# roboterax/humanoid-gym

Hardware: AMD Instinct MI355X
Metric: env-steps/s (XBot-L PPO, whole job) (higher is better)
Workload: dtype bf16

## Files before the change

humanoid-gym_amd/csrc/hgym_gae.hip:

```cpp
#include "hgym_common.hpp"

namespace hgym {

constexpr int GAE_ENVS = 16;
constexpr int GAE_PAD = 17;

template <bool BOOT>
__global__ __launch_bounds__(256) void gae_kernel(int T, int N, float* __restrict__ rewards,
                                                  const float* __restrict__ values, const uint8_t* __restrict__ dones,
                                                  const uint8_t* __restrict__ time_outs,
                                                  const float* __restrict__ last_values, float gamma, float lam,
                                                  float* __restrict__ returns, float* __restrict__ advantages,
                                                  double* __restrict__ stats) {
    __shared__ float s_r[64][GAE_PAD];
    __shared__ float s_v[65][GAE_PAD];
    __shared__ float s_d[64][GAE_PAD];
    __shared__ float s_carry[GAE_ENVS];
    __shared__ double s_sum[4][2];
    const int tid = threadIdx.x, lane = tid & 63, wave = tid >> 6;
    const int e0 = blockIdx.x * GAE_ENVS;
    const int nE = min(GAE_ENVS, N - e0);
    if (tid < GAE_ENVS) s_carry[tid] = 0.0f;
    double sum1 = 0.0, sum2 = 0.0;
    const int ntiles = (T + 63) / 64;
    for (int tile = ntiles - 1; tile >= 0; --tile) {
        const int t0 = tile * 64;
        const int nT = min(64, T - t0);
        __syncthreads();
        for (int i = tid; i < 65 * GAE_ENVS; i += 256) {
            const int t = i / GAE_ENVS, el = i % GAE_ENVS;
            if (el < nE) {
                const int tg = t0 + t;
                if (t < nT) {
                    const int64_t gi = (int64_t)tg * N + e0 + el;
                    const float v = values[gi];
                    float r = rewards[gi];
                    if (BOOT) {
                        const float to = (float)(time_outs[gi] != 0);
                        r = r + gamma * (v * to);
                        rewards[gi] = r;
                    }
                    s_r[t][el] = r;
                    s_d[t][el] = (float)dones[gi];
                    s_v[t][el] = v;
                } else if (t == nT) {
                    s_v[t][el] = (tg >= T) ? last_values[e0 + el] : values[(int64_t)tg * N + e0 + el];
                }
            }
        }
        __syncthreads();
        for (int q = 0; q < GAE_ENVS / 4; ++q) {
            const int el = wave * (GAE_ENVS / 4) + q;
            if (el >= nE) break;
            const bool valid = lane < nT;
            float a = 1.0f, b = 0.0f, v = 0.0f;
            if (valid) {
                v = s_v[lane][el];
                const float nt = 1.0f - s_d[lane][el];
                b = s_r[lane][el] + nt * gamma * s_v[lane + 1][el] - v;
                a = nt * gamma * lam;
            }
#pragma unroll
            for (int off = 1; off < 64; off <<= 1) {
                const float a2 = __shfl_down(a, off, 64);
                const float b2 = __shfl_down(b, off, 64);
                if (lane + off < 64) {
                    b = b + a * b2;
                    a = a * a2;
                }
            }
            const float carry = s_carry[el];
            const float adv_t = b + a * carry;
            const float ret = adv_t + v;
            const float adv = ret - v;
            const float head = __shfl(adv_t, 0, 64);
            if (valid) {
                s_r[lane][el] = ret;
                s_d[lane][el] = adv;
                sum1 += (double)adv;
                sum2 += (double)adv * (double)adv;
            }
            if (lane == 0) s_carry[el] = head;
        }
        __syncthreads();
        for (int i = tid; i < 64 * GAE_ENVS; i += 256) {
            const int t = i / GAE_ENVS, el = i % GAE_ENVS;
            if (t < nT && el < nE) {
                returns[(int64_t)(t0 + t) * N + e0 + el] = s_r[t][el];
                advantages[(int64_t)(t0 + t) * N + e0 + el] = s_d[t][el];
            }
        }
    }
#pragma unroll
    for (int off = 32; off > 0; off >>= 1) {
        sum1 += __shfl_down(sum1, off, 64);
        sum2 += __shfl_down(sum2, off, 64);
    }
    if (lane == 0) {
        s_sum[wave][0] = sum1;
        s_sum[wave][1] = sum2;
    }
    __syncthreads();
    __shared__ int s_last;
    double* __restrict__ part = stats + 4;
    unsigned int* cnt = reinterpret_cast<unsigned int*>(stats + 3);
    if (tid == 0) {
        part[2 * blockIdx.x] = s_sum[0][0] + s_sum[1][0] + s_sum[2][0] + s_sum[3][0];
        part[2 * blockIdx.x + 1] = s_sum[0][1] + s_sum[1][1] + s_sum[2][1] + s_sum[3][1];
        __builtin_amdgcn_fence(__ATOMIC_RELEASE, "agent");
        const unsigned int done = __hip_atomic_fetch_add(cnt, 1u, __ATOMIC_ACQ_REL, __HIP_MEMORY_SCOPE_AGENT);
        s_last = (done == gridDim.x - 1u) ? 1 : 0;
    }
    __syncthreads();
    if (s_last) {
        __builtin_amdgcn_fence(__ATOMIC_ACQUIRE, "agent");
        double a = 0.0, b = 0.0;
        for (int i = tid; i < (int)gridDim.x; i += 256) {
            a += part[2 * i];
            b += part[2 * i + 1];
        }
#pragma unroll
        for (int off = 32; off > 0; off >>= 1) {
            a += __shfl_down(a, off, 64);
            b += __shfl_down(b, off, 64);
        }
        __syncthreads();
        if (lane == 0) {
            s_sum[wave][0] = a;
            s_sum[wave][1] = b;
        }
        __syncthreads();
        if (tid == 0) {
            stats[0] = s_sum[0][0] + s_sum[1][0] + s_sum[2][0] + s_sum[3][0];
            stats[1] = s_sum[0][1] + s_sum[1][1] + s_sum[2][1] + s_sum[3][1];
            stats[2] = (double)T * (double)N;
            __hip_atomic_store(cnt, 0u, __ATOMIC_RELAXED, __HIP_MEMORY_SCOPE_AGENT);
        }
    }
}

__global__ __launch_bounds__(256) void adv_normalize_kernel(int64_t count, float* __restrict__ adv, const double* __restrict__ stats) {
    const double n = stats[2];
    const double mean_d = stats[0] / n;
    double var = (stats[1] - stats[0] * stats[0] / n) / (n - 1.0);
    if (var < 0.0) var = 0.0;
    const float mean = (float)mean_d;
    const float denom = (float)sqrt(var) + 1e-8f;
    for (int64_t i = (int64_t)blockIdx.x * blockDim.x + threadIdx.x; i < count; i += (int64_t)gridDim.x * blockDim.x)
        adv[i] = (adv[i] - mean) / denom;
}

__global__ __launch_bounds__(256) void store_step_kernel(int n, const float* __restrict__ rew, const float* __restrict__ values,
                                                         const uint8_t* __restrict__ time_outs, const uint8_t* __restrict__ dones,
                                                         float gamma, float* __restrict__ rewards_slot, uint8_t* __restrict__ dones_slot) {
    const int i = blockIdx.x * blockDim.x + threadIdx.x;
    if (i >= n) return;
    const float to = time_outs ? (float)(time_outs[i] != 0) : 0.0f;
    rewards_slot[i] = rew[i] + gamma * (values[i] * to);
    dones_slot[i] = dones[i] != 0;
}

HG_HD uint32_t perm_mix(uint32_t x) {
    x ^= x >> 16;
    x *= 0x7feb352du;
    x ^= x >> 15;
    x *= 0x846ca68bu;
    x ^= x >> 16;
    return x;
}
HG_HD uint64_t perm_key(uint64_t seed, uint64_t draw) { return (seed ^ (draw * 0x9e3779b97f4a7c15ull)) * 0xd1342543de82ef95ull + draw; }
HG_HD int64_t perm_index(int64_t i, int64_t n, int half_bits, uint32_t k0, uint32_t k1) {
    const uint32_t mask = (1u << half_bits) - 1u;
    uint64_t x = (uint64_t)i;
    do {
        uint32_t l = (uint32_t)(x >> half_bits) & mask, r = (uint32_t)x & mask;
#pragma unroll
        for (uint32_t round = 0; round < 6; ++round) {
            const uint32_t f = perm_mix(r ^ perm_mix(k0 + round * 0x9e3779b9u) ^ k1) & mask;
            const uint32_t t = l ^ f;
            l = r;
            r = t;
        }
        x = ((uint64_t)l << half_bits) | r;
    } while (x >= (uint64_t)n);
    return (int64_t)x;
}
__global__ __launch_bounds__(256) void randperm_kernel(int64_t n, int half_bits, uint32_t k0, uint32_t k1, int64_t* __restrict__ out) {
    for (int64_t i = (int64_t)blockIdx.x * blockDim.x + threadIdx.x; i < n; i += (int64_t)gridDim.x * blockDim.x)
        out[i] = perm_index(i, n, half_bits, k0, k1);
}

__global__ __launch_bounds__(256) void randperm_dev_kernel(int64_t n, int half_bits, uint64_t seed, const int64_t* __restrict__ draw_p,
                                                           int64_t* __restrict__ out) {
    const uint64_t draw = (uint64_t)draw_p[0];
    const uint64_t key = perm_key(seed, draw);
    const uint32_t k0 = (uint32_t)key, k1 = (uint32_t)(key >> 32);
    for (int64_t i = (int64_t)blockIdx.x * blockDim.x + threadIdx.x; i < n; i += (int64_t)gridDim.x * blockDim.x)
        out[i] = perm_index(i, n, half_bits, k0, k1);
}

}

using namespace hgym;

extern "C" {

int32_t hgym_randperm_dev(int64_t n, uint64_t seed, const int64_t* draw, int64_t* out, void* stream) {
    HG_REQUIRE(n > 0 && n <= ((int64_t)1 << 40), HGYM_E_SHAPE, "n=%lld", (long long)n);
    HG_REQUIRE(out && draw, HGYM_E_BADARG, "null pointer");
    int half_bits = 1;
    while (((int64_t)1 << (2 * half_bits)) < n) ++half_bits;
    const int blocks = (int)((n + 255) / 256 > 4096 ? 4096 : (n + 255) / 256);
    hipLaunchKernelGGL(randperm_dev_kernel, dim3(blocks), dim3(256), 0, (hipStream_t)stream, n, half_bits, seed, draw, out);
    HG_CHECK_LAUNCH("randperm_dev_kernel");
    return HGYM_OK;
}

int32_t hgym_randperm(int64_t n, uint64_t seed, uint64_t draw, int64_t* out, void* stream) {
    HG_REQUIRE(n > 0 && n <= ((int64_t)1 << 40), HGYM_E_SHAPE, "n=%lld", (long long)n);
    HG_REQUIRE(out, HGYM_E_BADARG, "null output");
    int half_bits = 1;
    while (((int64_t)1 << (2 * half_bits)) < n) ++half_bits;
    const uint64_t key = perm_key(seed, draw);
    const int blocks = (int)((n + 255) / 256 > 4096 ? 4096 : (n + 255) / 256);
    hipLaunchKernelGGL(randperm_kernel, dim3(blocks), dim3(256), 0, (hipStream_t)stream, n, half_bits, (uint32_t)key, (uint32_t)(key >> 32), out);
    HG_CHECK_LAUNCH("randperm_kernel");
    return HGYM_OK;
}

int32_t hgym_store_step(int32_t n, const float* rew, const float* values, const uint8_t* time_outs, const uint8_t* dones,
                        float gamma, float* rewards_slot, uint8_t* dones_slot, void* stream) {
    HG_REQUIRE(n > 0, HGYM_E_SHAPE, "n=%d", n);
    HG_REQUIRE(rew && values && dones && rewards_slot && dones_slot, HGYM_E_BADARG, "null pointer");
    hipLaunchKernelGGL(store_step_kernel, dim3(ceil_div(n, 256)), dim3(256), 0, (hipStream_t)stream, n, rew, values, time_outs, dones,
                       gamma, rewards_slot, dones_slot);
    HG_CHECK_LAUNCH("store_step_kernel");
    return HGYM_OK;
}

int32_t hgym_gae(int32_t T, int32_t n, const float* rewards, const float* values, const uint8_t* dones, const float* last_values,
                 float gamma, float lam, float* returns, float* advantages, double* stats, void* stream) {
    HG_REQUIRE(T > 0 && n > 0, HGYM_E_SHAPE, "T=%d n=%d", T, n);
    HG_REQUIRE(rewards && values && dones && last_values && returns && advantages && stats, HGYM_E_BADARG, "null pointer");
    prof_begin(HGYM_PROF_GAE, (hipStream_t)stream);
    hipLaunchKernelGGL(gae_kernel<false>, dim3(ceil_div(n, GAE_ENVS)), dim3(256), 0, (hipStream_t)stream, T, n, const_cast<float*>(rewards), values,
                       dones, nullptr, last_values, gamma, lam, returns, advantages, stats);
    prof_end(HGYM_PROF_GAE, (hipStream_t)stream, (double)T * n * 17.0);
    HG_CHECK_LAUNCH("gae_kernel");
    return HGYM_OK;
}

int32_t hgym_gae_bootstrap(int32_t T, int32_t n, float* rewards, const float* values, const uint8_t* dones, const uint8_t* time_outs,
                           const float* last_values, float gamma, float lam, float* returns, float* advantages, double* stats, void* stream) {
    HG_REQUIRE(T > 0 && n > 0, HGYM_E_SHAPE, "T=%d n=%d", T, n);
    HG_REQUIRE(rewards && values && dones && time_outs && last_values && returns && advantages && stats, HGYM_E_BADARG, "null pointer");
    prof_begin(HGYM_PROF_GAE, (hipStream_t)stream);
    hipLaunchKernelGGL(gae_kernel<true>, dim3(ceil_div(n, GAE_ENVS)), dim3(256), 0, (hipStream_t)stream, T, n, rewards, values, dones, time_outs,
                       last_values, gamma, lam, returns, advantages, stats);
    prof_end(HGYM_PROF_GAE, (hipStream_t)stream, (double)T * n * 22.0);
    HG_CHECK_LAUNCH("gae_kernel<bootstrap>");
    return HGYM_OK;
}

int32_t hgym_adv_normalize(int64_t count, float* advantages, const double* stats, void* stream) {
    HG_REQUIRE(count > 1, HGYM_E_SHAPE, "count=%lld", (long long)count);
    HG_REQUIRE(advantages && stats, HGYM_E_BADARG, "null pointer");
    const int blocks = (int)((count + 255) / 256 > 2048 ? 2048 : (count + 255) / 256);
    hipLaunchKernelGGL(adv_normalize_kernel, dim3(blocks), dim3(256), 0, (hipStream_t)stream, count, advantages, stats);
    HG_CHECK_LAUNCH("adv_normalize_kernel");
    return HGYM_OK;
}

}
```

humanoid-gym_amd/csrc/hgym_net.hip:

```cpp
#include <stdlib.h>

#include "hgym_gemm.hpp"
#include "hgym_fused.hpp"

namespace hgym {

int32_t launch_mlp_fb(const FwdArgs& fb, const FbLoss& fl, bool shadow, bool unclipped, int tiles, int nets, size_t lds, hipStream_t s);

struct LayerLayout {
    int K, N;
    int Kp, Ncp, N16, K16;
    int64_t w_off, b_off;
    int64_t Wp, WTp;
    int64_t X, XT, dY, dYT;
    int KBf, NBf, NBBf;
    int64_t Wf, WTf;
};

struct NetLayout {
    int L;
    bool fused;
    LayerLayout layer[HGYM_MAX_LAYERS];
    int64_t out_f32;
    int64_t X0b, Hb[3], dZb[4];
// ... 335 lines not shown
        } else {
#pragma unroll
            for (int j = 0; j < 16; ++j) {
                if (j >= A) continue;
                rowm[j] = a.mu[(int64_t)i * A + j];
                rowa[j] = a.b.actions[r * A + j];
                rowmo[j] = a.b.mu[r * A + j];
                rowso[j] = a.b.sigma[r * A + j];
            }
        }
#pragma unroll
        for (int j = 0; j < 16; ++j) {
            diff[j] = 0.0f;
            sg[j] = 1.0f;
            if (j >= A) continue;
            const float m = rowm[j];
            const float s = m * 0.0f + a.std_[j];
            const float act = rowa[j];
            const float mo = rowmo[j], so = rowso[j];
            const float d = act - m;
            diff[j] = d;
            sg[j] = s;
            lp += -(d * d) / (2.0f * s * s) - logf(s) - 0.9189385332046727f;
            ent += 0.5f + 0.9189385332046727f + logf(s);
            kl += logf(s / so + 1.e-5f) + (so * so + (mo - m) * (mo - m)) / (2.0f * (s * s)) - 0.5f;
        }
        const float ratio = expf(lp - lpold);
        const float s1 = -adv * ratio;
        const float s2 = -adv * clampf(ratio, 1.0f - a.clip, 1.0f + a.clip);
        const float surr = fmaxf(s1, s2);
        const float in_range = (ratio >= 1.0f - a.clip && ratio <= 1.0f + a.clip) ? 1.0f : 0.0f;
        const float w1 = s1 > s2 ? 1.0f : (s1 == s2 ? 0.5f : 0.0f);
        const float d_lp = (-adv) * (w1 + (1.0f - w1) * in_range) * invB * ratio;
        float vl, d_v;
        if constexpr (VU) {
            vl = (v - ret) * (v - ret);
            d_v = a.value_coef * invB * (2.0f * (v - ret));
        } else {
            const float vc = vold + clampf(v - vold, -a.clip, a.clip);
            const float l1 = (v - ret) * (v - ret), l2 = (vc - ret) * (vc - ret);
            vl = fmaxf(l1, l2);
            const float v_in = ((v - vold) >= -a.clip && (v - vold) <= a.clip) ? 1.0f : 0.0f;
            const float u1 = l1 > l2 ? 1.0f : (l1 == l2 ? 0.5f : 0.0f);
            d_v = a.value_coef * invB * (u1 * 2.0f * (v - ret) + (1.0f - u1) * 2.0f * (vc - ret) * v_in);
        }
#pragma unroll
        for (int j = 0; j < 16; ++j) {
            if (j >= A) continue;
            const float s = sg[j], d = diff[j];
            const float g_mu = d_lp * d / (s * s);
            const float g_sg = d_lp * (d * d / (s * s * s) - 1.0f / s) - (a.entropy_coef * invB) / s;
            if (j < 12) {
                acc[4 + j] = g_sg;
                acc[16 + j] = g_mu;
            }
            dmu[(int64_t)i * a.ld_dmu + j] = from_f32<T>(g_mu);
            dmuT[(int64_t)j * a.ld_t + i] = from_f32<T>(g_mu);
        }
        dval[(int64_t)i * a.ld_dval] = from_f32<T>(d_v);
        dvalT[i] = from_f32<T>(d_v);
        acc[0] = surr;
        acc[1] = vl;
        acc[2] = ent;
        acc[3] = kl;
        acc[28] = d_v;
    } else if (i < a.Bp) {
        for (int j = 0; j < A; ++j) dmuT[(int64_t)j * a.ld_t + i] = from_f32<T>(0.0f);
        dvalT[i] = from_f32<T>(0.0f);
    }
#pragma unroll
    for (int k = 0; k < LOSS_PARTIALS; ++k) {
        float s = acc[k];
#pragma unroll
        for (int off = 32; off > 0; off >>= 1) s += __shfl_down(s, off, 64);
        if ((threadIdx.x & 63) == 0) red[threadIdx.x >> 6][k] = s;
    }
    __syncthreads();
    if (threadIdx.x < LOSS_PARTIALS) a.partials[(int64_t)blockIdx.x * LOSS_PARTIALS + threadIdx.x] =
        red[0][threadIdx.x] + red[1][threadIdx.x] + red[2][threadIdx.x] + red[3][threadIdx.x];
}

__global__ __launch_bounds__(512) void ppo_scalars_kernel(const ScalArgs a) { ppo_scalars_block(a, threadIdx.x, blockDim.x); }

struct Segment {
    int64_t off;
    int rows, cols;
    int splits;
    void* Wp;
    int64_t ldw;
    void* WTp;
    int64_t ldwt;
    void* Wf;
    void* WTf;
    int KB, NBB;
};
struct SegTable {
    int n;
    Segment s[2 * HGYM_MAX_LAYERS * 2 + 1];
};

__global__ __launch_bounds__(256) void reduce_slabs_kernel(const SegTable tab, int64_t P, const float* __restrict__ slabs,
                                                           float* __restrict__ grads, double* __restrict__ opt) {
    __shared__ double red[4];
    const Segment& sg = tab.s[blockIdx.y];
    const int64_t n = (int64_t)sg.rows * sg.cols;
    const int64_t stride = (int64_t)gridDim.x * blockDim.x;
    double sq = 0.0;
    if (sg.splits == 0) {
        for (int64_t i = (int64_t)blockIdx.x * blockDim.x + threadIdx.x; i < n; i += stride) {
            const float g = grads[sg.off + i];
            sq += (double)g * (double)g;
        }
    } else {
        const bool vec = (P & 3) == 0 && (((uintptr_t)grads | (uintptr_t)slabs) & 15) == 0;
        const int64_t head = vec ? ((4 - (sg.off & 3)) & 3) < n ? ((4 - (sg.off & 3)) & 3) : n : n;
        const int64_t n4 = (n - head) >> 2, tail0 = head + 4 * n4;
        const int64_t base = sg.off + head;
        for (int64_t i = (int64_t)blockIdx.x * blockDim.x + threadIdx.x; i < n4; i += stride) {
            float4 acc = make_float4(0.f, 0.f, 0.f, 0.f);
            if (sg.splits == 8) {
                float4 v[8];
#pragma unroll
                for (int z = 0; z < 8; ++z) v[z] = *reinterpret_cast<const float4*>(slabs + (int64_t)z * P + base + 4 * i);
#pragma unroll
                for (int z = 0; z < 8; ++z) { acc.x += v[z].x; acc.y += v[z].y; acc.z += v[z].z; acc.w += v[z].w; }
            } else {
                for (int z = 0; z < sg.splits; ++z) {
                    const float4 v = *reinterpret_cast<const float4*>(slabs + (int64_t)z * P + base + 4 * i);
                    acc.x += v.x; acc.y += v.y; acc.z += v.z; acc.w += v.w;
                }
            }
            *reinterpret_cast<float4*>(grads + base + 4 * i) = acc;
            sq += (double)acc.x * (double)acc.x + (double)acc.y * (double)acc.y + (double)acc.z * (double)acc.z + (double)acc.w * (double)acc.w;
        }
        for (int64_t i = (int64_t)blockIdx.x * blockDim.x + threadIdx.x; i < head + (n - tail0); i += stride) {
            const int64_t e = i < head ? i : tail0 + (i - head);
            float s = 0.0f;
            for (int z = 0; z < sg.splits; ++z) s += slabs[(int64_t)z * P + sg.off + e];
            grads[sg.off + e] = s;
            sq += (double)s * (double)s;
        }
    }
#pragma unroll
    for (int off = 32; off > 0; off >>= 1) sq += __shfl_down(sq, off, 64);
    if ((threadIdx.x & 63) == 0) red[threadIdx.x >> 6] = sq;
    __syncthreads();
    if (threadIdx.x == 0) {
        double t = red[0] + red[1] + red[2] + red[3];
        t = __builtin_rint(t * 0x1p46) * 0x1p-46;
        if (t != 0.0) atomicAdd(&opt[9], t);
    }
}


__device__ __forceinline__ void apply_prologue(const HgymPPOConfig& p, const float* __restrict__ kl_slot, float inv_w, double* __restrict__ opt,
                                               int have_sq, double sq) {
    if (p.world_size > 1) opt[8] = (double)(kl_slot[0] * inv_w);
    if (opt[13] == opt[1] && opt[1] > 0.0) {
        if (have_sq >= 0) opt[9] = have_sq ? sq : 0.0;
        return;
    }
    if (p.adaptive_lr) opt[0] = adapt_lr(opt[0], (float)opt[8], p.desired_kl, p.lr_min, p.lr_max);
    const double t = opt[1] + 1.0;
    opt[1] = t;
    const bool cached = opt[13] == t;
    const double bc1 = 1.0 - (cached ? opt[14] : pow((double)p.beta1, t)), bc2 = 1.0 - (cached ? opt[15] : pow((double)p.beta2, t));
    opt[11] = (double)(float)(opt[0] / bc1);
    opt[12] = (double)(float)sqrt(bc2);
    opt[13] = t;
    if (have_sq >= 0) opt[9] = have_sq ? sq : 0.0;
}
__global__ void apply_prologue_kernel(const HgymPPOConfig p, const float* __restrict__ kl_slot, float inv_w, double* __restrict__ opt) {
    if (threadIdx.x != 0 || blockIdx.x != 0) return;
    apply_prologue(p, kl_slot, inv_w, opt, (p.world_size > 1 || !p.grad_norm_ready) ? 0 : -1, 0.0);
}

__global__ __launch_bounds__(256) void sqnorm_prologue_kernel(int64_t P, const float* __restrict__ g, float inv_w, const HgymPPOConfig p,
                                                              const float* __restrict__ kl_slot, double* __restrict__ opt,
                                                              double* __restrict__ part) {
    __shared__ double red[4];
    __shared__ unsigned int s_last;
    double s = 0.0;
    for (int64_t i = (int64_t)blockIdx.x * blockDim.x + threadIdx.x; i < P; i += (int64_t)gridDim.x * blockDim.x) {
        const float gi = g[i] * inv_w;
        s += (double)gi * (double)gi;
    }
#pragma unroll
    for (int off = 32; off > 0; off >>= 1) s += __shfl_down(s, off, 64);
    if ((threadIdx.x & 63) == 0) red[threadIdx.x >> 6] = s;
    __syncthreads();
    unsigned int* counter = reinterpret_cast<unsigned int*>(part + SQN_BLOCKS);
    if (threadIdx.x == 0) {
        part[blockIdx.x] = red[0] + red[1] + red[2] + red[3];
        __threadfence();
        s_last = atomicAdd(counter, 1u) == gridDim.x - 1u ? 1u : 0u;
    }
    __syncthreads();
    if (!s_last) return;
    __threadfence();
    double v = threadIdx.x < gridDim.x ? reinterpret_cast<const volatile double*>(part)[threadIdx.x] : 0.0;
#pragma unroll
    for (int off = 32; off > 0; off >>= 1) v += __shfl_down(v, off, 64);
    __syncthreads();
    if ((threadIdx.x & 63) == 0) red[threadIdx.x >> 6] = v;
    __syncthreads();
    if (threadIdx.x == 0) {
        *counter = 0u;
        apply_prologue(p, kl_slot, inv_w, opt, 1, red[0] + red[1] + red[2] + red[3]);
    }
}

template <typename T>
__device__ __forceinline__ void write_shadows(const Segment& sg, int r, int c, float w) {
    if (sg.Wp) {
        ((T*)sg.Wp)[(int64_t)r * sg.ldw + c] = from_f32<T>(w);
        if (sg.WTp) ((T*)sg.WTp)[(int64_t)c * sg.ldwt + r] = from_f32<T>(w);
    }
    if (sg.Wf) {
        ((T*)sg.Wf)[((((int64_t)(r >> 4) * sg.KB + (c >> 5)) * 64) + ((c & 31) >> 3) * 16 + (r & 15)) * 8 + (c & 7)] = from_f32<T>(w);
        ((T*)sg.WTf)[((((int64_t)(c >> 4) * sg.NBB + (r >> 5)) * 64) + ((r & 31) >> 3) * 16 + (c & 15)) * 8 + (r & 7)] = from_f32<T>(w);
    }
}

template <typename T>
__global__ __launch_bounds__(256) void adam_kernel(const SegTable tab, const HgymPPOConfig p, float* __restrict__ params,
                                                   float* __restrict__ grads, float* __restrict__ m_, float* __restrict__ v_,
                                                   float inv_w, double* __restrict__ opt) {
    const Segment& sg = tab.s[blockIdx.y];
    const int64_t n = (int64_t)sg.rows * sg.cols;
    const float total = (float)sqrt(opt[9]);
    float coef = p.max_grad_norm / (total + 1e-6f);
    coef = fminf(coef, 1.0f);
    if (blockIdx.x == 0 && blockIdx.y == 0 && threadIdx.x == 0) {
        opt[6] = (double)total;
        opt[13] = -1.0;
    }
    const float step_size = (float)opt[11], sqrt_bc2 = (float)opt[12];
    auto adam1 = [&](int64_t q) -> float {
        const float g = (grads[q] * inv_w) * coef;
        grads[q] = g;
        const float m = m_[q] * p.beta1 + (1.0f - p.beta1) * g;
        const float v = v_[q] * p.beta2 + (1.0f - p.beta2) * (g * g);
        m_[q] = m;
        v_[q] = v;
        const float denom = sqrtf(v) / sqrt_bc2 + p.adam_eps;
        const float w = params[q] + (-step_size * m) / denom;
        params[q] = w;
        return w;
    };
    for (int64_t i = (int64_t)blockIdx.x * blockDim.x + threadIdx.x; i < n; i += (int64_t)gridDim.x * blockDim.x) {
        const float w = adam1(sg.off + i);
        if (sg.Wp || sg.Wf) {
            const int r = (int)(i / sg.cols), c = (int)(i - (int64_t)r * sg.cols);
            write_shadows<T>(sg, r, c, w);
        }
    }
}

template <typename T>
__global__ __launch_bounds__(256) void sync_shadow_kernel(const SegTable tab, const float* __restrict__ params) {
    const Segment& sg = tab.s[blockIdx.y];
    if (!sg.Wp && !sg.Wf) return;
    const int64_t n = (int64_t)sg.rows * sg.cols;
    for (int64_t i = (int64_t)blockIdx.x * blockDim.x + threadIdx.x; i < n; i += (int64_t)gridDim.x * blockDim.x) {
        const int r = (int)(i / sg.cols), c = (int)(i - (int64_t)r * sg.cols);
        write_shadows<T>(sg, r, c, params[sg.off + i]);
    }
}

template <typename T, int BM, int BN, int WMs, int WNs>
static void launch_cfg(const GemmArgs& g, int splits, hipStream_t s) {
    constexpr int F = ((BM / 16) + (BN / 16)) * KSTAGE;
    constexpr size_t lds = (size_t)2 * F * 1024;
    (void)ensure_dynamic_lds(reinterpret_cast<const void*>(&gemm_nt_kernel<T, BM, BN, WMs, WNs>), lds, "gemm_nt_kernel");
    dim3 grid(ceil_div(g.N, BN), ceil_div(g.M, BM), splits);
    hipLaunchKernelGGL((gemm_nt_kernel<T, BM, BN, WMs, WNs>), grid, dim3(WMs * WNs * 64), lds, s, g);
}

template <typename T>
int32_t launch_gemm(const GemmArgs& g0, int splits, hipStream_t s) {
    GemmArgs g = g0;
    constexpr int SE = stage_elems<T>();
    HG_REQUIRE(g.K % SE == 0 && g.K > 0, HGYM_E_SHAPE, "gemm K=%d not a multiple of %d", g.K, SE);
    HG_REQUIRE(g.lda * (int64_t)sizeof(T) % 16 == 0 && g.ldb * (int64_t)sizeof(T) % 16 == 0, HGYM_E_SHAPE, "gemm operand rows must be 16-byte aligned");
    if (splits < 1) splits = 1;
    int stages = g.K / SE;
    if (splits > stages) splits = stages;
    const int per = ceil_div(stages, splits);
    splits = ceil_div(stages, per);
    g.k_chunk = per * SE;
    prof_begin(HGYM_PROF_GEMM, s);
    const int64_t t128 = (int64_t)ceil_div(g.M, 128) * ceil_div(g.N, 128) * splits;
    if (g.N <= 16) launch_cfg<T, 128, 16, 4, 1>(g, splits, s);
    else if (g.M <= 16) launch_cfg<T, 16, 128, 1, 4>(g, splits, s);
    else if (t128 >= 192) launch_cfg<T, 128, 128, 2, 2>(g, splits, s);
    else launch_cfg<T, 64, 64, 2, 2>(g, splits, s);
    prof_end(HGYM_PROF_GEMM, s, 2.0 * (double)g.M * (double)g.N * (double)g.K);
    HG_CHECK_LAUNCH("gemm_nt_kernel");
    return splits;
}

struct NetIO {
    const float* x;
    int64_t ldx;
    float* out;
    int64_t ldo;
};

static int64_t shadow_ld(const WsLayout& w, int which) { return (int64_t)w.net[which].layer[0].KBf * 32; }

static int32_t check_shadow(const WsLayout& w, const HgymObsShadow* sh) {
    if (!sh) return HGYM_OK;
    HG_REQUIRE((!sh->obs || (sh->ld_obs >= shadow_ld(w, 0) && sh->ld_obs % 8 == 0 && ((uintptr_t)sh->obs & 15) == 0)) &&
                   (!sh->priv || (sh->ld_priv >= shadow_ld(w, 1) && sh->ld_priv % 8 == 0 && ((uintptr_t)sh->priv & 15) == 0)),
               HGYM_E_SHAPE, "observation shadow: leading dimensions %lld / %lld (need >= %lld / %lld, multiples of 8, 16-byte aligned rows)",
               (long long)sh->ld_obs, (long long)sh->ld_priv, (long long)shadow_ld(w, 0), (long long)shadow_ld(w, 1));
    return HGYM_OK;
}

static size_t fwd_lds(const FwdArgs& a, int nets, int BM) {
    size_t lds = 0;
    for (int i = 0; i < nets; ++i) lds = std::max(lds, (size_t)fwd_lds_bytes(a.net[a.net0 + i], BM));
    return lds;
}

struct NetBase {
    const HgymNetConfig& cfg;
    const HgymNet& net;
    const WsLayout& w;
    hipStream_t s;
    char* ws;

    template <typename U> U* at(int64_t off) const { return reinterpret_cast<U*>(ws + off); }

    int split_count(const LayerLayout& y, int Mp) const {
        const int tiles = ceil_div(y.N, y.N <= 16 ? 16 : 128) * ceil_div(y.K, 128);
        int sp = ceil_div(512, tiles);
        if (sp > w.splits) sp = w.splits;
        const int stages = Mp / w.SE;
        if (sp > stages) sp = stages;
        if (sp < 1) sp = 1;
        const int per = ceil_div(stages, sp);
        return ceil_div(stages, per);
    }

    int rowsum_splits(int Mp, int* per_out = nullptr) const {
        const int chunks = ceil_div(Mp, 1024 * 16 / w.es);
        const int per = ceil_div(chunks, std::min(chunks, w.splits));
        if (per_out) *per_out = per;
        return ceil_div(chunks, per);
    }

    SegTable segments(int Mp) const {
        SegTable t;
        memset(&t, 0, sizeof(t));
        Segment& sd = t.s[t.n++];
        sd.off = 0;
        sd.rows = cfg.num_actions;
        sd.cols = 1;
        for (int which = 0; which < w.nnets; ++which) {
            const NetLayout& n = w.net[which];
            for (int l = 0; l < n.L; ++l) {
                const LayerLayout& y = n.layer[l];
                Segment& a = t.s[t.n++];
                a.off = y.w_off;
                a.rows = y.N;
                a.cols = y.K;
                if (n.fused) {
                    a.splits = Mp ? w.dw_splits : 0;
                    a.Wf = ws + y.Wf;
                    a.WTf = ws + y.WTf;
                    a.KB = y.KBf;
                    a.NBB = y.NBBf;
                } else {
                    a.splits = Mp ? split_count(y, Mp) : 0;
                    a.Wp = ws + y.Wp;
                    a.ldw = y.Kp;
                    a.WTp = ws + y.WTp;
                    a.ldwt = y.Ncp;
                }
                Segment& b = t.s[t.n++];
                b.off = y.b_off;
                b.rows = y.N;
                b.cols = 1;
                if (n.fused && Mp && (l < n.L - 1 || which == 2)) b.splits = w.dw_splits;
                if (!n.fused && Mp) b.splits = rowsum_splits(Mp);
            }
        }
        return t;
    }

    template <typename T>
    int32_t apply(const HgymPPOConfig& ppo, bool prologue_done) {
        prof_begin(HGYM_PROF_APPLY, s);
        const float inv_w = ppo.world_size > 1 ? (float)(1.0 / (double)ppo.world_size) : 1.0f;
        if (ppo.world_size > 1 || !ppo.grad_norm_ready)
            hipLaunchKernelGGL(sqnorm_prologue_kernel, dim3(SQN_BLOCKS), dim3(256), 0, s, w.P, net.grads, inv_w, ppo, net.grads + w.P, net.opt_state,
                               at<double>(w.sqn));
        else if (!prologue_done)
            hipLaunchKernelGGL(apply_prologue_kernel, dim3(1), dim3(64), 0, s, ppo, net.grads + w.P, inv_w, net.opt_state);
        const SegTable tab = segments(0);
        hipLaunchKernelGGL((adam_kernel<T>), dim3(256, tab.n), dim3(256), 0, s, tab, ppo, net.params, net.grads, net.adam_m, net.adam_v,
                           inv_w, net.opt_state);
        prof_end(HGYM_PROF_APPLY, s, (double)w.P * 36.0);
        HG_CHECK_LAUNCH("adam_kernel");
        return HGYM_OK;
    }

    template <typename T>
    int32_t sync_shadow() {
        const SegTable tab = segments(0);
        hipLaunchKernelGGL((sync_shadow_kernel<T>), dim3(64, tab.n), dim3(256), 0, s, tab, net.params);
        HG_CHECK_LAUNCH("sync_shadow_kernel");
        return HGYM_OK;
    }
};

template <typename T>
struct GemmPath : NetBase {
    int32_t forward(int which, int M, const float* x, int64_t ldx, const int64_t* idx, float* y_out, int64_t ld_out, bool train) {
        const NetLayout& n = w.net[which];
        HG_REQUIRE(M > 0 && M <= w.maxM, HGYM_E_SHAPE, "batch %d exceeds max_batch %lld", M, (long long)w.maxM);
        const LayerLayout& l0 = n.layer[0];
        const int64_t total = (int64_t)M * l0.K;
        hipLaunchKernelGGL((pack_rows_kernel<T>), dim3((int)std::min<int64_t>(ceil_div(total, 256), 4096)), dim3(256), 0, s, M, l0.K, x,
                           ldx, idx, at<T>(l0.X), (int64_t)l0.Kp);
        HG_CHECK_LAUNCH("pack_rows_kernel");
        const int Mp = (int)round_up(M, w.SE);
        for (int l = 0; l < n.L; ++l) {
            const LayerLayout& y = n.layer[l];
            const bool last = l == n.L - 1;
            if (train) {
                hipLaunchKernelGGL((transpose_kernel<T>), dim3(ceil_div(Mp, 64), ceil_div(y.K, 64)), dim3(256), 0, s, M, Mp, y.K,
                                   at<T>(y.X), (int64_t)y.Kp, at<T>(y.XT), w.Mp);
                HG_CHECK_LAUNCH("transpose_kernel");
            }
            GemmArgs g;
            memset(&g, 0, sizeof(g));
            g.A = at<T>(y.X);
            g.lda = y.Kp;
            g.rowsA = M;
            g.B = at<T>(y.Wp);
            g.ldb = y.Kp;
            g.rowsB = y.N16;
            g.M = M;
            g.N = y.N;
            g.K = y.Kp;
            g.bias = net.params + y.b_off;
            if (last) {
                g.Cf = y_out;
                g.ldcf = ld_out;
            } else {
                g.act = ACT_APPLY;
                g.fn = w.act;
                g.Ct = at<T>(n.layer[l + 1].X);
                g.ldct = n.layer[l + 1].Kp;
            }
            const int32_t rc = launch_gemm<T>(g, 1, s);
            if (rc < 0) return rc;
        }
        return HGYM_OK;
    }

    int32_t backward(int which, int M) {
        const NetLayout& n = w.net[which];
        const int Mp = (int)round_up(M, w.SE);
        for (int l = n.L - 1; l >= 0; --l) {
            const LayerLayout& y = n.layer[l];
            {
                GemmArgs g;
                memset(&g, 0, sizeof(g));
                g.A = at<T>(y.dYT);
                g.lda = w.Mp;
                g.rowsA = y.N16;
                g.B = at<T>(y.XT);
                g.ldb = w.Mp;
                g.rowsB = y.K16;
                g.M = y.N;
                g.N = y.K;
                g.K = Mp;
                g.Cf = at<float>(w.slabs) + y.w_off;
                g.ldcf = y.K;
                g.slab_stride = w.Ps;
                const int want = split_count(y, Mp);
                const int32_t got = launch_gemm<T>(g, want, s);
                if (got < 0) return got;
                HG_REQUIRE(got == want, HGYM_E_LAUNCH, "split-K mismatch %d vs %d", got, want);
                int per = 0;
                const int rs = rowsum_splits(Mp, &per);
                hipLaunchKernelGGL((rowsum_kernel<T>), dim3(rs, y.N), dim3(256), 0, s, Mp, per, at<T>(y.dYT), w.Mp,
                                   at<float>(w.slabs) + y.b_off, w.Ps);
                HG_CHECK_LAUNCH("rowsum_kernel");
            }
            if (l > 0) {
                const LayerLayout& p = n.layer[l - 1];
                GemmArgs g;
                memset(&g, 0, sizeof(g));
                g.A = at<T>(y.dY);
                g.lda = y.Ncp;
                g.rowsA = M;
                g.B = at<T>(y.WTp);
                g.ldb = y.Ncp;
                g.rowsB = y.K16;
                g.M = M;
                g.N = y.K;
                g.K = y.Ncp;
                g.aux = at<T>(y.X);
                g.ldaux = y.Kp;
                g.fn = w.act;
                g.Ct = at<T>(p.dY);
                g.ldct = p.Ncp;
                const int32_t rc = launch_gemm<T>(g, 1, s);
                if (rc < 0) return rc;
                hipLaunchKernelGGL((transpose_kernel<T>), dim3(ceil_div(Mp, 64), ceil_div(p.N, 64)), dim3(256), 0, s, M, Mp, p.N,
                                   at<T>(p.dY), (int64_t)p.Ncp, at<T>(p.dYT), w.Mp);
                HG_CHECK_LAUNCH("transpose_kernel");
            }
        }
        return HGYM_OK;
    }

    int32_t aux_grad(const HgymPPOConfig& ppo, const HgymBatch& b) {
        const NetLayout& n = w.net[2];
        const LayerLayout& last = n.layer[n.L - 1];
        const int B = b.B, No = last.N;
        float* y = at<float>(n.out_f32);
        int32_t rc = forward(2, B, b.obs, cfg.num_obs, b.idx, y, No, true);
        if (rc) return rc;
        const int Bp = (int)round_up(B, w.SE);
        hipLaunchKernelGGL((aux_mse_kernel<T>), dim3(ceil_div(Bp, 256)), dim3(256), 0, s, B, Bp, No, y, b.priv, (int64_t)cfg.num_priv,
                           cfg.aux_target_offset, b.idx, ppo.aux_coef, at<T>(last.dY), (int64_t)last.Ncp, at<T>(last.dYT), w.Mp,
                           net.opt_state);
        HG_CHECK_LAUNCH("aux_mse_kernel");
        return backward(2, B);
    }

    int32_t grad(const HgymPPOConfig& ppo, const HgymBatch& b, int part) {
        if (part == 1) return HGYM_OK;
        const int B = b.B, A = cfg.num_actions;
        float* mu = at<float>(w.net[0].out_f32);
        float* val = at<float>(w.net[1].out_f32);
        int32_t rc = forward(0, B, b.obs, cfg.num_obs, b.idx, mu, A, true);
        if (rc) return rc;
        rc = forward(1, B, b.priv, cfg.num_priv, b.idx, val, 1, true);
        if (rc) return rc;
        const int Bp = (int)round_up(B, w.SE);
        const int nblocks = ceil_div(Bp, 256);
        HG_REQUIRE(nblocks <= MAX_LOSS_BLOCKS, HGYM_E_UNSUPPORTED, "minibatch %d too large for the loss partial buffer", B);
        const LayerLayout& la = w.net[0].layer[w.net[0].L - 1];
        const LayerLayout& lc = w.net[1].layer[w.net[1].L - 1];
        LossArgs a;
        memset(&a, 0, sizeof(a));
        a.b = b;
        a.A = A;
        a.mu = mu;
        a.val = val;
// ... 534 lines not shown
```

Baseline: 43.16 million.

## Vectorize GAE kernel and flatten Adam grid with tiled fragment-shadow writes

Adds a GAE kernel that handles twice as many envs per 512-thread block and loads and stores rewards, values, dones and time-outs as float4/uint32 vectors. It writes per-virtual-block partial sums so the existing stats layout is kept. The Adam launch becomes a flat 1D grid sized per segment instead of a fixed 256-by-segments grid. For bf16 fragment-layout shadows it stages updated weights through LDS tiles and writes packed 16-byte fragments for both the weight and its transpose, replacing scattered element writes. Both paths fall back to the old kernels through env vars or when alignment checks fail, at the cost of extra code complexity and LDS use.

```diff
diff --git a/humanoid-gym_amd/csrc/hgym_gae.hip b/humanoid-gym_amd/csrc/hgym_gae.hip
--- a/humanoid-gym_amd/csrc/hgym_gae.hip
+++ b/humanoid-gym_amd/csrc/hgym_gae.hip
@@ -139,6 +139,161 @@
     }
 }
 
+constexpr int GAEV_ENVS = 2 * GAE_ENVS;
+constexpr int GAEV_PAD = GAEV_ENVS + 1;
+template <bool BOOT>
+__global__ __launch_bounds__(512) void gae_vec_kernel(int T, int N, float* __restrict__ rewards, const float* __restrict__ values,
+                                                      const uint8_t* __restrict__ dones, const uint8_t* __restrict__ time_outs,
+                                                      const float* __restrict__ last_values, float gamma, float lam,
+                                                      float* __restrict__ returns, float* __restrict__ advantages, double* __restrict__ stats) {
+    __shared__ float s_r[64][GAEV_PAD];
+    __shared__ float s_v[65][GAEV_PAD];
+    __shared__ float s_d[64][GAEV_PAD];
+    __shared__ float s_carry[GAEV_ENVS];
+    __shared__ double s_sum[8][2];
+    const int tid = threadIdx.x, lane = tid & 63, wave = tid >> 6;
+    const int e0 = blockIdx.x * GAEV_ENVS;
+    const int nE = min(GAEV_ENVS, N - e0);
+    const int nvirt = (N + GAE_ENVS - 1) / GAE_ENVS;
+    const int st = tid >> 3, sg = (tid & 7) * 4;
+    if (tid < GAEV_ENVS) s_carry[tid] = 0.0f;
+    double sum1 = 0.0, sum2 = 0.0;
+    const int ntiles = (T + 63) / 64;
+    for (int tile = ntiles - 1; tile >= 0; --tile) {
+        const int t0 = tile * 64;
+        const int nT = min(64, T - t0);
+        const bool mine = st < nT && sg < nE;
+        const int64_t gi = (int64_t)(t0 + st) * N + e0 + sg;
+        float4 r4 = make_float4(0.f, 0.f, 0.f, 0.f), v4 = r4, x4 = r4;
+        uint32_t d4 = 0, to4 = 0;
+        if (mine) {
+            v4 = *reinterpret_cast<const float4*>(values + gi);
+            r4 = *reinterpret_cast<const float4*>(rewards + gi);
+            d4 = *reinterpret_cast<const uint32_t*>(dones + gi);
+            if (BOOT) to4 = *reinterpret_cast<const uint32_t*>(time_outs + gi);
+        }
+        const bool next = tid < GAEV_ENVS / 4 && tid * 4 < nE;
+        if (next)
+            x4 = (t0 + nT >= T) ? *reinterpret_cast<const float4*>(last_values + e0 + tid * 4)
+                                : *reinterpret_cast<const float4*>(values + (int64_t)(t0 + nT) * N + e0 + tid * 4);
+        __syncthreads();
+        if (mine) {
+            const float rr[4] = {r4.x, r4.y, r4.z, r4.w}, vv[4] = {v4.x, v4.y, v4.z, v4.w};
+            float ro[4];
+#pragma unroll
+            for (int j = 0; j < 4; ++j) {
+                float r = rr[j];
+                if (BOOT) {
+                    const float to = (float)(((to4 >> (8 * j)) & 0xffu) != 0);
+                    r = r + gamma * (vv[j] * to);
+                }
+                ro[j] = r;
+                s_r[st][sg + j] = r;
+                s_d[st][sg + j] = (float)((d4 >> (8 * j)) & 0xffu);
+                s_v[st][sg + j] = vv[j];
+            }
+            if (BOOT) *reinterpret_cast<float4*>(rewards + gi) = make_float4(ro[0], ro[1], ro[2], ro[3]);
+        }
+        if (next) {
+            s_v[nT][tid * 4 + 0] = x4.x;
+            s_v[nT][tid * 4 + 1] = x4.y;
+            s_v[nT][tid * 4 + 2] = x4.z;
+            s_v[nT][tid * 4 + 3] = x4.w;
+        }
+        __syncthreads();
+        for (int q = 0; q < GAE_ENVS / 4; ++q) {
+            const int el = (wave >> 2) * GAE_ENVS + (wave & 3) * (GAE_ENVS / 4) + q;
+            if (el >= nE) break;
+            const bool valid = lane < nT;
+            float a = 1.0f, b = 0.0f, v = 0.0f;
+            if (valid) {
+                v = s_v[lane][el];
+                const float nt = 1.0f - s_d[lane][el];
+                b = s_r[lane][el] + nt * gamma * s_v[lane + 1][el] - v;
+                a = nt * gamma * lam;
+            }
+#pragma unroll
+            for (int off = 1; off < 64; off <<= 1) {
+                const float a2 = __shfl_down(a, off, 64);
+                const float b2 = __shfl_down(b, off, 64);
+                if (lane + off < 64) {
+                    b = b + a * b2;
+                    a = a * a2;
+                }
+            }
+            const float carry = s_carry[el];
+            const float adv_t = b + a * carry;
+            const float ret = adv_t + v;
+            const float adv = ret - v;
+            const float head = __shfl(adv_t, 0, 64);
+            if (valid) {
+                s_r[lane][el] = ret;
+                s_d[lane][el] = adv;
+                sum1 += (double)adv;
+                sum2 += (double)adv * (double)adv;
+            }
+            if (lane == 0) s_carry[el] = head;
+        }
+        __syncthreads();
+        if (mine) {
+            *reinterpret_cast<float4*>(returns + gi) = make_float4(s_r[st][sg], s_r[st][sg + 1], s_r[st][sg + 2], s_r[st][sg + 3]);
+            *reinterpret_cast<float4*>(advantages + gi) = make_float4(s_d[st][sg], s_d[st][sg + 1], s_d[st][sg + 2], s_d[st][sg + 3]);
+        }
+    }
+#pragma unroll
+    for (int off = 32; off > 0; off >>= 1) {
+        sum1 += __shfl_down(sum1, off, 64);
+        sum2 += __shfl_down(sum2, off, 64);
+    }
+    if (lane == 0) {
+        s_sum[wave][0] = sum1;
+        s_sum[wave][1] = sum2;
+    }
+    __syncthreads();
+    __shared__ int s_last;
+    double* __restrict__ part = stats + 4;
+    unsigned int* cnt = reinterpret_cast<unsigned int*>(stats + 3);
+    if (tid == 0) {
+        for (int h = 0; h < 2; ++h) {
+            const int vb = 2 * blockIdx.x + h;
+            if (vb >= nvirt) break;
+            part[2 * vb] = s_sum[4 * h][0] + s_sum[4 * h + 1][0] + s_sum[4 * h + 2][0] + s_sum[4 * h + 3][0];
+            part[2 * vb + 1] = s_sum[4 * h][1] + s_sum[4 * h + 1][1] + s_sum[4 * h + 2][1] + s_sum[4 * h + 3][1];
+        }
+        __builtin_amdgcn_fence(__ATOMIC_RELEASE, "agent");
+        const unsigned int done = __hip_atomic_fetch_add(cnt, 1u, __ATOMIC_ACQ_REL, __HIP_MEMORY_SCOPE_AGENT);
+        s_last = (done == gridDim.x - 1u) ? 1 : 0;
+    }
+    __syncthreads();
+    if (s_last) {
+        __builtin_amdgcn_fence(__ATOMIC_ACQUIRE, "agent");
+        double a = 0.0, b = 0.0;
+        if (tid < 256) {
+            for (int i = tid; i < nvirt; i += 256) {
+                a += part[2 * i];
+                b += part[2 * i + 1];
+            }
+        }
+#pragma unroll
+        for (int off = 32; off > 0; off >>= 1) {
+            a += __shfl_down(a, off, 64);
+            b += __shfl_down(b, off, 64);
+        }
+        __syncthreads();
+        if (lane == 0) {
+            s_sum[wave][0] = a;
+            s_sum[wave][1] = b;
+        }
+        __syncthreads();
+        if (tid == 0) {
+            stats[0] = s_sum[0][0] + s_sum[1][0] + s_sum[2][0] + s_sum[3][0];
+            stats[1] = s_sum[0][1] + s_sum[1][1] + s_sum[2][1] + s_sum[3][1];
+            stats[2] = (double)T * (double)N;
+            __hip_atomic_store(cnt, 0u, __ATOMIC_RELAXED, __HIP_MEMORY_SCOPE_AGENT);
+        }
+    }
+}
+
 __global__ __launch_bounds__(256) void adv_normalize_kernel(int64_t count, float* __restrict__ adv, const double* __restrict__ stats) {
     const double n = stats[2];
     const double mean_d = stats[0] / n;
@@ -203,6 +358,14 @@
 
 using namespace hgym;
 
+static bool gae_vec_ok(int n, const float* rewards, const float* values, const uint8_t* dones, const uint8_t* time_outs, const float* last_values,
+                       const float* returns, const float* advantages) {
+    if (getenv("HGYM_GAE_OLD") || (n & 3)) return false;
+    const uintptr_t f = (uintptr_t)rewards | (uintptr_t)values | (uintptr_t)last_values | (uintptr_t)returns | (uintptr_t)advantages;
+    const uintptr_t b = (uintptr_t)dones | (uintptr_t)time_outs;
+    return (f & 15) == 0 && (b & 3) == 0;
+}
+
 extern "C" {
 
 int32_t hgym_randperm_dev(int64_t n, uint64_t seed, const int64_t* draw, int64_t* out, void* stream) {
@@ -243,8 +406,12 @@
     HG_REQUIRE(T > 0 && n > 0, HGYM_E_SHAPE, "T=%d n=%d", T, n);
     HG_REQUIRE(rewards && values && dones && last_values && returns && advantages && stats, HGYM_E_BADARG, "null pointer");
     prof_begin(HGYM_PROF_GAE, (hipStream_t)stream);
-    hipLaunchKernelGGL(gae_kernel<false>, dim3(ceil_div(n, GAE_ENVS)), dim3(256), 0, (hipStream_t)stream, T, n, const_cast<float*>(rewards), values,
-                       dones, nullptr, last_values, gamma, lam, returns, advantages, stats);
+    if (gae_vec_ok(n, rewards, values, dones, nullptr, last_values, returns, advantages))
+        hipLaunchKernelGGL(gae_vec_kernel<false>, dim3(ceil_div(n, GAEV_ENVS)), dim3(512), 0, (hipStream_t)stream, T, n, const_cast<float*>(rewards),
+                           values, dones, nullptr, last_values, gamma, lam, returns, advantages, stats);
+    else
+        hipLaunchKernelGGL(gae_kernel<false>, dim3(ceil_div(n, GAE_ENVS)), dim3(256), 0, (hipStream_t)stream, T, n, const_cast<float*>(rewards), values,
+                           dones, nullptr, last_values, gamma, lam, returns, advantages, stats);
     prof_end(HGYM_PROF_GAE, (hipStream_t)stream, (double)T * n * 17.0);
     HG_CHECK_LAUNCH("gae_kernel");
     return HGYM_OK;
@@ -255,8 +422,12 @@
     HG_REQUIRE(T > 0 && n > 0, HGYM_E_SHAPE, "T=%d n=%d", T, n);
     HG_REQUIRE(rewards && values && dones && time_outs && last_values && returns && advantages && stats, HGYM_E_BADARG, "null pointer");
     prof_begin(HGYM_PROF_GAE, (hipStream_t)stream);
-    hipLaunchKernelGGL(gae_kernel<true>, dim3(ceil_div(n, GAE_ENVS)), dim3(256), 0, (hipStream_t)stream, T, n, rewards, values, dones, time_outs,
-                       last_values, gamma, lam, returns, advantages, stats);
+    if (gae_vec_ok(n, rewards, values, dones, time_outs, last_values, returns, advantages))
+        hipLaunchKernelGGL(gae_vec_kernel<true>, dim3(ceil_div(n, GAEV_ENVS)), dim3(512), 0, (hipStream_t)stream, T, n, rewards, values, dones,
+                           time_outs, last_values, gamma, lam, returns, advantages, stats);
+    else
+        hipLaunchKernelGGL(gae_kernel<true>, dim3(ceil_div(n, GAE_ENVS)), dim3(256), 0, (hipStream_t)stream, T, n, rewards, values, dones, time_outs,
+                           last_values, gamma, lam, returns, advantages, stats);
     prof_end(HGYM_PROF_GAE, (hipStream_t)stream, (double)T * n * 22.0);
     HG_CHECK_LAUNCH("gae_kernel<bootstrap>");
     return HGYM_OK;
diff --git a/humanoid-gym_amd/csrc/hgym_net.hip b/humanoid-gym_amd/csrc/hgym_net.hip
--- a/humanoid-gym_amd/csrc/hgym_net.hip
+++ b/humanoid-gym_amd/csrc/hgym_net.hip
@@ -511,6 +511,15 @@
     }
 }
 
+struct SegGrid {
+    int first[2 * HGYM_MAX_LAYERS * 2 + 2];
+};
+__device__ __forceinline__ int seg_of(const SegGrid& g, int n, int b) {
+    int s = 0;
+    while (s + 1 < n && b >= g.first[s + 1]) ++s;
+    return s;
+}
+
 
 __device__ __forceinline__ void apply_prologue(const HgymPPOConfig& p, const float* __restrict__ kl_slot, float inv_w, double* __restrict__ opt,
                                                int have_sq, double sq) {
@@ -614,6 +623,121 @@
             write_shadows<T>(sg, r, c, w);
         }
     }
+}
+
+constexpr int ADAM_UR = 16, ADAM_UC = 32;
+template <typename T>
+__global__ __launch_bounds__(256) void adam_flat_kernel(const SegTable tab, const SegGrid grid, const HgymPPOConfig p, float* __restrict__ params,
+                                                        float* __restrict__ grads, float* __restrict__ m_, float* __restrict__ v_,
+                                                        float inv_w, double* __restrict__ opt, int frag) {
+    const int seg = seg_of(grid, tab.n, blockIdx.x);
+    const Segment& sg = tab.s[seg];
+    const int x = blockIdx.x - grid.first[seg], nx = grid.first[seg + 1] - grid.first[seg];
+    const int64_t n = (int64_t)sg.rows * sg.cols;
+    const float total = (float)sqrt(opt[9]);
+    float coef = p.max_grad_norm / (total + 1e-6f);
+    coef = fminf(coef, 1.0f);
+    if (blockIdx.x == 0 && threadIdx.x == 0) {
+        opt[6] = (double)total;
+        opt[13] = -1.0;
+    }
+    const float step_size = (float)opt[11], sqrt_bc2 = (float)opt[12];
+    auto adam_math = [&](float g0, float m0, float v0, float w0, float& g, float& m, float& v) -> float {
+        g = (g0 * inv_w) * coef;
+        m = m0 * p.beta1 + (1.0f - p.beta1) * g;
+        v = v0 * p.beta2 + (1.0f - p.beta2) * (g * g);
+        const float denom = sqrtf(v) / sqrt_bc2 + p.adam_eps;
+        return w0 + (-step_size * m) / denom;
+    };
+    auto adam1 = [&](int64_t q) -> float {
+        float g, m, v;
+        const float w = adam_math(grads[q], m_[q], v_[q], params[q], g, m, v);
+        grads[q] = g;
+        m_[q] = m;
+        v_[q] = v;
+        params[q] = w;
+        return w;
+    };
+    if constexpr (sizeof(T) == 2) {
+        if (frag && sg.Wf) {
+            __shared__ float s_tile[4][ADAM_UR][ADAM_UC + 1];
+            const int lane = threadIdx.x & 63, wave = threadIdx.x >> 6;
+            float(*tile)[ADAM_UC + 1] = s_tile[wave];
+            const int cbn = (sg.cols + ADAM_UC - 1) / ADAM_UC, units = ((sg.rows + ADAM_UR - 1) / ADAM_UR) * cbn;
+            const int lr = lane >> 5, lc = lane & 31;
+            for (int u = x * 4 + wave; u < units; u += nx * 4) {
+                const int r0 = (u / cbn) * ADAM_UR, c0 = (u % cbn) * ADAM_UC;
+                if (r0 + ADAM_UR <= sg.rows && c0 + ADAM_UC <= sg.cols) {
+                    const int64_t q0 = sg.off + (int64_t)(r0 + lr) * sg.cols + c0 + lc;
+                    float g0[8], m0[8], v0[8], w0[8];
+#pragma unroll
+                    for (int i = 0; i < 8; ++i) {
+                        const int64_t q = q0 + (int64_t)(2 * i) * sg.cols;
+                        g0[i] = grads[q];
+                        m0[i] = m_[q];
+                        v0[i] = v_[q];
+                        w0[i] = params[q];
+                    }
+#pragma unroll
+                    for (int i = 0; i < 8; ++i) {
+                        const int64_t q = q0 + (int64_t)(2 * i) * sg.cols;
+                        float g, m, v;
+                        const float w = adam_math(g0[i], m0[i], v0[i], w0[i], g, m, v);
+                        grads[q] = g;
+                        m_[q] = m;
+                        v_[q] = v;
+                        params[q] = w;
+                        tile[2 * i + lr][lc] = w;
+                    }
+                    asm volatile("s_waitcnt lgkmcnt(0)" ::: "memory");
+                    __builtin_amdgcn_wave_barrier();
+                    struct alignas(16) Pack8 { T e[8]; };
+                    Pack8 pk;
+                    {
+                        const int r = lane & 15, cq = lane >> 4;
+#pragma unroll
+                        for (int j = 0; j < 8; ++j) pk.e[j] = from_f32<T>(tile[r][cq * 8 + j]);
+                        *reinterpret_cast<Pack8*>((T*)sg.Wf + (((int64_t)(r0 >> 4) * sg.KB + (c0 >> 5)) * 64 + lane) * 8) = pk;
+                    }
+                    {
+                        const int cl = (lane >> 5) * 16 + (lane & 15), rq = (lane >> 4) & 1;
+#pragma unroll
+                        for (int j = 0; j < 8; ++j) pk.e[j] = from_f32<T>(tile[rq * 8 + j][cl]);
+                        const int r = r0 + rq * 8, c = c0 + cl;
+                        *reinterpret_cast<Pack8*>((T*)sg.WTf + ((((int64_t)(c >> 4) * sg.NBB + (r >> 5)) * 64) + ((r & 31) >> 3) * 16 + (c & 15)) * 8) = pk;
+                    }
+                    asm volatile("s_waitcnt lgkmcnt(0)" ::: "memory");
+                    __builtin_amdgcn_wave_barrier();
+                } else {
+#pragma unroll 1
+                    for (int i = 0; i < 8; ++i) {
+                        const int r = r0 + 2 * i + lr, c = c0 + lc;
+                        if (r < sg.rows && c < sg.cols) write_shadows<T>(sg, r, c, adam1(sg.off + (int64_t)r * sg.cols + c));
+                    }
+                }
+            }
+            return;
+        }
+    }
+    for (int64_t i = (int64_t)x * blockDim.x + threadIdx.x; i < n; i += (int64_t)nx * blockDim.x) {
+        const float w = adam1(sg.off + i);
+        if (sg.Wp || sg.Wf) {
+            const int r = (int)(i / sg.cols), c = (int)(i - (int64_t)r * sg.cols);
+            write_shadows<T>(sg, r, c, w);
+        }
+    }
+}
+
+static SegGrid adam_grid(const SegTable& tab, bool frag) {
+    SegGrid g;
+    memset(&g, 0, sizeof(g));
+    for (int s = 0; s < tab.n; ++s) {
+        const Segment& sg = tab.s[s];
+        const int64_t n = (int64_t)sg.rows * sg.cols;
+        const int64_t wg = frag && sg.Wf ? ((int64_t)ceil_div(sg.rows, ADAM_UR) * ceil_div(sg.cols, ADAM_UC) + 3) / 4 : std::min<int64_t>(256, (n + 1023) / 1024);
+        g.first[s + 1] = g.first[s] + (int)std::max<int64_t>(1, wg);
+    }
+    return g;
 }
 
 template <typename T>
@@ -759,8 +883,16 @@
         else if (!prologue_done)
             hipLaunchKernelGGL(apply_prologue_kernel, dim3(1), dim3(64), 0, s, ppo, net.grads + w.P, inv_w, net.opt_state);
         const SegTable tab = segments(0);
-        hipLaunchKernelGGL((adam_kernel<T>), dim3(256, tab.n), dim3(256), 0, s, tab, ppo, net.params, net.grads, net.adam_m, net.adam_v,
-                           inv_w, net.opt_state);
+        const char* old = getenv("HGYM_ADAM_OLD");
+        if (old && old[0] == '1') {
+            hipLaunchKernelGGL((adam_kernel<T>), dim3(256, tab.n), dim3(256), 0, s, tab, ppo, net.params, net.grads, net.adam_m, net.adam_v,
+                               inv_w, net.opt_state);
+        } else {
+            const bool frag = !old;
+            const SegGrid grid = adam_grid(tab, frag);
+            hipLaunchKernelGGL((adam_flat_kernel<T>), dim3(grid.first[tab.n]), dim3(256), 0, s, tab, grid, ppo, net.params, net.grads, net.adam_m,
+                               net.adam_v, inv_w, net.opt_state, frag ? 1 : 0);
+        }
         prof_end(HGYM_PROF_APPLY, s, (double)w.P * 36.0);
         HG_CHECK_LAUNCH("adam_kernel");
         return HGYM_OK;
```

New measurement: 43.26 million (median of 6 runs). No clear change (+0.2%).
